# AssemblyAI-Community/MinImagen

Measured on NVIDIA H100. Metric: denoising steps/sec (SR256 U-Net, batch 32 per GPU per step), higher is better.
Workload: dtype f16 tensor-core operands, f32 accumulate / residual stream

## Files before the change

### minimagen_b200/csrc/conv_tc.cu

```cuda
#include "conv_tc.cuh"

#include <cuda_runtime.h>
#include <mutex>
#include <stdio.h>

#include "kernels.cuh"
#include "launch.cuh"
#include "ptx.cuh"
#include "sat_half.cuh"
#include "wgmma.cuh"

namespace mi {

namespace {

constexpr int kNumThreads = 384;
constexpr uint32_t kABytes = kConvBlockM * kConvBlockK * 2;
constexpr uint32_t kRingBudget = 192 * 1024;
constexpr uint32_t kAuxBytes = 512;
constexpr uint32_t kSmemMax = 227 * 1024;
constexpr int kProducerRegs = 40;
constexpr int kConsumerRegs = 232;
static_assert(128 * kProducerRegs + 256 * kConsumerRegs <= 65536, "register file overcommitted");
constexpr int kTurnBar = 2;
constexpr int kStatBar = 4;
constexpr uint32_t stat_scratch_bytes(int block_n) { return 2 * 4 * (block_n / 16 > 0 ? block_n / 16 : 1) * 2 * 8; }

template <int BLOCK_N>
struct Cfg {
    static constexpr uint32_t kBBytes = BLOCK_N * kConvBlockK * 2;
    static constexpr uint32_t kStageBytes = kABytes + kBBytes;
    static constexpr int kStages = (kRingBudget / kStageBytes) > 8 ? 8 : (kRingBudget / kStageBytes);
    static constexpr uint32_t kSmemBytes = kStages * kStageBytes + 1024  + kAuxBytes;
};

__device__ __forceinline__ float silu(float v) { return __fdividef(v, 1.0f + __expf(-v)); }

template <int BLOCK_N, bool GN>
__global__ void __launch_bounds__(kNumThreads, 1)
conv_wg_kernel(const __grid_constant__ CUtensorMap tmA, const __grid_constant__ CUtensorMap tmA2,
               const __grid_constant__ CUtensorMap tmB, const __grid_constant__ CUtensorMap tmX,
               const __grid_constant__ CUtensorMap tmX2, const __grid_constant__ ConvTcArgs args,
               const __grid_constant__ GnPrologueArgs gn) {
    using C = Cfg<BLOCK_N>;
    constexpr int STAGES = C::kStages;
    static_assert(2 * STAGES * 8 <= 256, "barrier block overlaps the GroupNorm scratch");
    constexpr bool PP = !GN && BLOCK_N <= 128;
    constexpr int HALVES = PP ? 2 : 1;

    extern __shared__ uint8_t smem_raw[];
    uint8_t* smem = reinterpret_cast<uint8_t*>((reinterpret_cast<uintptr_t>(smem_raw) + 1023) & ~uintptr_t(1023));
    uint64_t* bars = reinterpret_cast<uint64_t*>(smem + STAGES * C::kStageBytes);
    uint64_t* full_bar = bars;
    uint64_t* empty_bar = bars + STAGES;

    const int warp = threadIdx.x >> 5;
    const int lane = threadIdx.x & 31;
    const int wg = threadIdx.x >> 7;
    int* err = args.err_flag;

    if (threadIdx.x == 0) {
        ptx::prefetch_tensormap(&tmB);
        if (!GN) {
            ptx::prefetch_tensormap(&tmA);
            ptx::prefetch_tensormap(&tmA2);
        }
        for (int i = 0; i < STAGES; ++i) {
            ptx::mbar_init(&full_bar[i], GN ? 5 : 1);
            ptx::mbar_init(&empty_bar[i], PP ? 1 : 2);
        }
        ptx::fence_barrier_init();
    }
    __syncthreads();
    pdl_wait();

    const int num_tap_kb = args.num_taps * args.chunks_per_tap;
    const int num_kb = num_tap_kb + args.x_chunks;
    const int tiles_m = args.tiles_w * args.tiles_h * args.tiles_b;
    const int total_tiles = tiles_m * args.tiles_n;
    const int BW = 1 << args.bw_log2, BH = 1 << args.bh_log2;
    const int BB = kConvBlockM >> (args.bw_log2 + args.bh_log2);

    if (wg == 0) {
        if constexpr (!GN) {
            ptx::setmaxnreg_dec<kProducerRegs>();
            if (warp == 0) {
                int stage = 0;
                uint32_t phase = 0;
                for (int tile = blockIdx.x; tile < total_tiles; tile += gridDim.x) {
                    const int nt = tile % args.tiles_n;
                    const int mt = tile / args.tiles_n;
                    const int w0 = (mt % args.tiles_w) * BW;
                    const int h0 = ((mt / args.tiles_w) % args.tiles_h) * BH;
                    const int b0 = (mt / (args.tiles_w * args.tiles_h)) * BB;
                    const int n0 = nt * BLOCK_N;
                    for (int kb = 0; kb < num_kb; ++kb) {
                        ptx::mbar_wait(&empty_bar[stage], phase ^ 1, err, 100 + stage);
                        if (ptx::elect_one()) {
                            uint8_t* sa = smem + stage * C::kStageBytes;
                            uint8_t* sb = sa + kABytes;
                            ptx::mbar_arrive_expect_tx(&full_bar[stage], C::kStageBytes);
                            if (kb < num_tap_kb) {
                                const int t = kb / args.chunks_per_tap, j = kb - t * args.chunks_per_tap;
                                const int cw = w0 * args.in_stride + args.dw[t], ch = h0 * args.in_stride + args.dh[t];
                                if (j < args.a_split)
                                    ptx::tma_load_5d(&tmA, &full_bar[stage], sa, args.a_chan_off + j * kConvBlockK, cw, ch,
                                                     args.ph[t], b0);
                                else
                                    ptx::tma_load_5d(&tmA2, &full_bar[stage], sa,
                                                     args.a_chan_off2 + (j - args.a_split) * kConvBlockK, cw, ch, args.ph[t], b0);
                            } else {
                                const int jx = kb - num_tap_kb;
                                if (jx < args.x_split)
                                    ptx::tma_load_5d(&tmX, &full_bar[stage], sa, args.x_chan_off + jx * kConvBlockK, w0, h0, 0, b0);
                                else
                                    ptx::tma_load_5d(&tmX2, &full_bar[stage], sa,
                                                     args.x_chan_off2 + (jx - args.x_split) * kConvBlockK, w0, h0, 0, b0);
                            }
                            ptx::tma_load_2d(&tmB, &full_bar[stage], sb, kb * kConvBlockK, n0);
                        }
                        if (++stage == STAGES) { stage = 0; phase ^= 1; }
                    }
                }
                pdl_trigger();
            }
        } else {
            float* s_mean = reinterpret_cast<float*>(reinterpret_cast<uint8_t*>(bars) + 256);
            float* s_rstd = s_mean + 32;
            float* sA = reinterpret_cast<float*>(reinterpret_cast<uint8_t*>(bars) + kAuxBytes);
            const int tt = threadIdx.x;
            const int lq = tt & 7;
            const int prow = tt >> 3;
            const int C0 = gn.C0, C1 = gn.C1, Ctot = C0 + C1, Cg = Ctot / gn.groups;
            const int H = args.H, W = args.W;
            float* sB = sA + Ctot;
            int stage = 0;
            uint32_t phase = 0;
            int cur_b = -1;
            for (int tile = blockIdx.x; tile < total_tiles; tile += gridDim.x) {
                const int nt = tile % args.tiles_n;
                const int mt = tile / args.tiles_n;
                const int w0 = (mt % args.tiles_w) * BW;
                const int h0 = ((mt / args.tiles_w) % args.tiles_h) * BH;
                const int b = mt / (args.tiles_w * args.tiles_h);
                const int n0 = nt * BLOCK_N;
                if (b != cur_b) {
                    ptx::bar_sync(1, 128);
                    if (tt < gn.groups) {
                        const int g = tt;
                        double su = 0.0, sq = 0.0;
                        const int lo = g * Cg, hi = lo + Cg;
                        const int lo0 = min(lo, C0), hi0 = min(hi, C0);
                        for (int e = lo0 / 16; e < hi0 / 16; ++e) {
                            su += gn.stats0[((long long)b * (C0 / 16) + e) * 2];
                            sq += gn.stats0[((long long)b * (C0 / 16) + e) * 2 + 1];
                        }
                        const int lo1 = max(lo, C0) - C0, hi1 = max(hi, C0) - C0;
                        for (int e = lo1 / 16; e < hi1 / 16; ++e) {
                            su += (double)gn.scale1 * gn.stats1[((long long)b * (C1 / 16) + e) * 2];
                            sq += (double)gn.scale1 * (double)gn.scale1 * gn.stats1[((long long)b * (C1 / 16) + e) * 2 + 1];
                        }
                        const double n = (double)Cg * H * W;
                        const double mean = su / n;
                        double var = sq / n - mean * mean;
                        if (var < 0) var = 0;
                        s_mean[g] = (float)mean;
                        s_rstd[g] = (float)(1.0 / sqrt(var + (double)gn.eps));
                    }
                    ptx::bar_sync(1, 128);
                    for (int cc = tt; cc < Ctot; cc += 128) {
                        const int g = cc / Cg;
                        float a = s_rstd[g] * gn.gamma[cc];
                        float bb = gn.beta[cc] - s_mean[g] * a;
                        if (gn.scale_shift) {
                            const float sc = gn.scale_shift[(long long)b * gn.ss_ld + cc] + 1.0f;
                            const float shv = gn.scale_shift[(long long)b * gn.ss_ld + Ctot + cc];
                            a *= sc;
                            bb = bb * sc + shv;
                        }
                        if (cc >= C0) a *= gn.scale1;
                        sA[cc] = a;
                        sB[cc] = bb;
                    }
                    cur_b = b;
                    ptx::bar_sync(1, 128);
                }
                const long long img = (long long)b * H * W;
                for (int kb = 0; kb < num_kb; ++kb) {
                    const int t = kb / args.chunks_per_tap, j = kb - t * args.chunks_per_tap;
                    const int dh = args.dh[t], dw = args.dw[t];
                    const float* cA = sA + j * kConvBlockK + lq * 8;
                    const float* cB = sB + j * kConvBlockK + lq * 8;
                    const float4 a0 = *reinterpret_cast<const float4*>(cA), a1 = *reinterpret_cast<const float4*>(cA + 4);
                    const float4 b0 = *reinterpret_cast<const float4*>(cB), b1 = *reinterpret_cast<const float4*>(cB + 4);
                    const bool first = j < args.a_split;
                    const int Cs = first ? C0 : C1;
                    const float* src = (first ? gn.src0 + (long long)j * kConvBlockK
                                              : gn.src1 + (long long)(j - args.a_split) * kConvBlockK) + img * Cs + lq * 8;

                    ptx::mbar_wait(&empty_bar[stage], phase ^ 1, err, 600 + stage);
                    uint8_t* sa = smem + stage * C::kStageBytes;
                    if (warp == 0 && ptx::elect_one()) {
                        ptx::mbar_arrive_expect_tx(&full_bar[stage], C::kBBytes);
                        ptx::tma_load_2d(&tmB, &full_bar[stage], sa + kABytes, kb * kConvBlockK, n0);
                    }
                    float4 x0[8], x1[8];
                    bool ok[8];
#pragma unroll
                    for (int i = 0; i < 8; ++i) {
                        const int m = i * 16 + prow;
                        const int gw = w0 + (m & (BW - 1)) + dw;
                        const int gh = h0 + ((m >> args.bw_log2) & (BH - 1)) + dh;
                        ok[i] = gh >= 0 && gh < H && gw >= 0 && gw < W;
                        if (ok[i]) {
                            const float4* s4 = reinterpret_cast<const float4*>(src + ((long long)gh * W + gw) * Cs);
                            x0[i] = __ldg(s4);
                            x1[i] = __ldg(s4 + 1);
                        }
                    }
#pragma unroll
                    for (int i = 0; i < 8; ++i) {
                        const int m = i * 16 + prow;
                        uint4 o = make_uint4(0u, 0u, 0u, 0u);
                        if (ok[i]) {
                            const __half2 h0_ = sat_half2(silu(fmaf(x0[i].x, a0.x, b0.x)), silu(fmaf(x0[i].y, a0.y, b0.y)));
                            const __half2 h1_ = sat_half2(silu(fmaf(x0[i].z, a0.z, b0.z)), silu(fmaf(x0[i].w, a0.w, b0.w)));
                            const __half2 h2_ = sat_half2(silu(fmaf(x1[i].x, a1.x, b1.x)), silu(fmaf(x1[i].y, a1.y, b1.y)));
                            const __half2 h3_ = sat_half2(silu(fmaf(x1[i].z, a1.z, b1.z)), silu(fmaf(x1[i].w, a1.w, b1.w)));
                            o.x = *reinterpret_cast<const uint32_t*>(&h0_); o.y = *reinterpret_cast<const uint32_t*>(&h1_);
                            o.z = *reinterpret_cast<const uint32_t*>(&h2_); o.w = *reinterpret_cast<const uint32_t*>(&h3_);
                        }
                        *reinterpret_cast<uint4*>(sa + m * 128 + ((lq ^ (m & 7)) << 4)) = o;
                    }
                    ptx::fence_proxy_async_smem();
                    __syncwarp();
                    if (lane == 0) ptx::mbar_arrive(&full_bar[stage]);
                    if (++stage == STAGES) { stage = 0; phase ^= 1; }
                }
            }
            pdl_trigger();
        }
    } else {
        if constexpr (!GN) ptx::setmaxnreg_inc<kConsumerRegs>();
        const int cw = wg - 1;
        const int wq = warp & 3;
        const int cq = 2 * (lane & 3);
        float acc[HALVES][BLOCK_N / 2];
        int stage = 0;
        uint32_t phase = 0;
        auto skip = [&](int n) {
            stage += n % STAGES;
            phase ^= (uint32_t)(n / STAGES) & 1u;
            if (stage >= STAGES) { stage -= STAGES; phase ^= 1; }
        };
        if (PP) skip(cw * num_kb);
        int bw_r[2 * HALVES], bh_r[2 * HALVES], bb_r[2 * HALVES], bb_warp[HALVES];
#pragma unroll
        for (int h = 0; h < HALVES; ++h) {
            const int m_warp = (PP ? h : cw) * 64 + wq * 16;
            bb_warp[h] = m_warp >> (args.bw_log2 + args.bh_log2);
#pragma unroll
            for (int r = 0; r < 2; ++r) {
                const int m = m_warp + (lane >> 2) + 8 * r;
                bw_r[2 * h + r] = m & (BW - 1);
                bh_r[2 * h + r] = (m >> args.bw_log2) & (BH - 1);
                bb_r[2 * h + r] = m >> (args.bw_log2 + args.bh_log2);
            }
        }
        constexpr int NQ = BLOCK_N / 16 > 0 ? BLOCK_N / 16 : 1;
        const bool tile_stats = PP && args.stats != nullptr && BB == 1;
        double* st_red = reinterpret_cast<double*>(reinterpret_cast<uint8_t*>(bars) + kAuxBytes);
        const bool vec = args.out_sc == 1 && ((reinterpret_cast<uintptr_t>(args.out_f32) & 7) == 0) &&
                         ((reinterpret_cast<uintptr_t>(args.residual) & 7) == 0) &&
                         ((reinterpret_cast<uintptr_t>(args.out_f16) & 3) == 0);

        for (int tile = blockIdx.x + (PP ? cw : 0) * gridDim.x; tile < total_tiles; tile += (PP ? 2 : 1) * gridDim.x) {
            const int nt = tile % args.tiles_n;
            const int mt = tile / args.tiles_n;
            const int n0 = nt * BLOCK_N;
            if (PP && tile != (int)blockIdx.x) ptx::bar_sync(kTurnBar + cw, 256);
            int prev = -1;
            for (int kb = 0; kb < num_kb; ++kb) {
                ptx::mbar_wait(&full_bar[stage], phase, err, 300 + stage);
                const uint32_t sa = ptx::smem_u32(smem + stage * C::kStageBytes);
                const uint64_t db = ptx::make_sw128_desc(sa + kABytes);
                ptx::wg_fence();
#pragma unroll
                for (int k = 0; k < kConvBlockK / 16; ++k)
#pragma unroll
                    for (int h = 0; h < HALVES; ++h) {
                        const uint64_t da = ptx::make_sw128_desc(sa + (PP ? h : cw) * (64 * 128));
                        ptx::Wgmma<BLOCK_N, 0>::run(acc[h], da + 2 * k, db + 2 * k, (kb | k) != 0);
                    }
                ptx::wg_commit();
                ptx::wg_wait<1>();
                if (prev >= 0 && (threadIdx.x & 127) == 0) ptx::mbar_arrive(&empty_bar[prev]);
                prev = stage;
                if (++stage == STAGES) { stage = 0; phase ^= 1; }
            }
            if (PP && tile + (int)gridDim.x < total_tiles) ptx::bar_arrive(kTurnBar + (cw ^ 1), 256);
            if (PP) skip(num_kb);
            ptx::wg_wait<0>();
#pragma unroll
            for (int h = 0; h < HALVES; ++h) ptx::wg_fence_regs(acc[h]);
            if (prev >= 0 && (threadIdx.x & 127) == 0) ptx::mbar_arrive(&empty_bar[prev]);

            const int tw0 = (mt % args.tiles_w) * BW;
            const int th0 = ((mt / args.tiles_w) % args.tiles_h) * BH;
            const int tb0 = (mt / (args.tiles_w * args.tiles_h)) * BB;
            const bool fast = vec && n0 + BLOCK_N <= args.n_valid;
#pragma unroll
            for (int hf = 0; hf < HALVES; ++hf) {
                bool valid[2];
                long long pix[2];
#pragma unroll
                for (int r = 0; r < 2; ++r) {
                    const int w = tw0 + bw_r[2 * hf + r], h = th0 + bh_r[2 * hf + r], b = tb0 + bb_r[2 * hf + r];
                    valid[r] = (b < args.B) && (h < args.H) && (w < args.W);
                    pix[r] = (long long)b * args.out_sb + (long long)h * args.out_sh + (long long)w * args.out_sw;
                }
                const float* a = acc[hf];
                float st_s[BLOCK_N / 16 > 0 ? BLOCK_N / 16 : 1], st_q[BLOCK_N / 16 > 0 ? BLOCK_N / 16 : 1];
#pragma unroll
                for (int q = 0; q < BLOCK_N / 16; ++q) { st_s[q] = 0.f; st_q[q] = 0.f; }
#pragma unroll
                for (int j = 0; j < BLOCK_N / 8; ++j) {
                    const int n = n0 + 8 * j + cq;
                    if (fast) {
                        float2 bv = make_float2(0.f, 0.f);
                        if (args.bias) bv = __ldg(reinterpret_cast<const float2*>(args.bias + n));
#pragma unroll
                        for (int r = 0; r < 2; ++r) {
                            if (!valid[r]) continue;
                            const long long o = pix[r] + n;
                            float2 f = make_float2(a[4 * j + 2 * r] + bv.x, a[4 * j + 2 * r + 1] + bv.y);
                            if (args.residual) {
                                const float2 rv = *reinterpret_cast<const float2*>(args.residual + o);
                                f.x += rv.x; f.y += rv.y;
                            }
                            st_s[j >> 1] += f.x + f.y;
                            st_q[j >> 1] += f.x * f.x + f.y * f.y;
                            if (args.out_f32) *reinterpret_cast<float2*>(args.out_f32 + o) = f;
                            if (args.out_f16) *reinterpret_cast<__half2*>(args.out_f16 + o) = sat_half2(f.x, f.y);
                        }
                    } else {
#pragma unroll
                        for (int r = 0; r < 2; ++r) {
#pragma unroll
                            for (int e = 0; e < 2; ++e) {
                                if (!valid[r] || n + e >= args.n_valid) continue;
                                float f = a[4 * j + 2 * r + e] + (args.bias ? __ldg(args.bias + n + e) : 0.f);
                                const long long o = pix[r] + (long long)(n + e) * args.out_sc;
                                if (args.residual && args.out_sc == 1) f += args.residual[o];
                                st_s[j >> 1] += f;
                                st_q[j >> 1] += f * f;
                                if (args.out_f32) args.out_f32[o] = f;
                                if (args.out_f16) args.out_f16[o] = sat_half(f);
                            }
                        }
                    }
                }
                if (args.stats) {
                    const int b_img = tb0 + bb_warp[hf];
                    const bool any = __any_sync(0xffffffffu, valid[0] || valid[1]);
#pragma unroll
                    for (int q = 0; q < BLOCK_N / 16; ++q) {
#pragma unroll
                        for (int o = 1; o <= 16; o <<= 1) {
                            st_s[q] += __shfl_xor_sync(0xffffffffu, st_s[q], o);
                            st_q[q] += __shfl_xor_sync(0xffffffffu, st_q[q], o);
                        }
                        if (lane == 0 && tile_stats) {
                            double* r = st_red + ((cw * 4 + wq) * NQ + q) * 2;
                            r[0] = (hf == 0 ? 0.0 : r[0]) + (double)st_s[q];
                            r[1] = (hf == 0 ? 0.0 : r[1]) + (double)st_q[q];
                        } else if (lane == 0 && any) {
                            double* dst = args.stats + ((long long)b_img * args.stats_blocks + (n0 >> 4) + q) * 2;
                            atomicAdd(dst, (double)st_s[q]);
                            atomicAdd(dst + 1, (double)st_q[q]);
                        }
                    }
                }
            }
            if (tile_stats) {
                ptx::bar_sync(kStatBar + cw, 128);
                if (wq == 0 && lane < NQ) {
                    const double* r = st_red + (cw * 4 * NQ + lane) * 2;
                    double s = r[0], sq = r[1];
#pragma unroll
                    for (int w = 1; w < 4; ++w) { s += r[w * NQ * 2]; sq += r[w * NQ * 2 + 1]; }
                    double* dst = args.stats + ((long long)tb0 * args.stats_blocks + (n0 >> 4) + lane) * 2;
                    atomicAdd(dst, s);
                    atomicAdd(dst + 1, sq);
                }
                ptx::bar_sync(kStatBar + cw, 128);
            }
        }
    }
}


typedef CUresult (*PFN_encodeTiled)(CUtensorMap*, CUtensorMapDataType, cuuint32_t, void*, const cuuint64_t*,
                                    const cuuint64_t*, const cuuint32_t*, const cuuint32_t*, CUtensorMapInterleave,
                                    CUtensorMapSwizzle, CUtensorMapL2promotion, CUtensorMapFloatOOBfill);

PFN_encodeTiled get_encode() {
    static PFN_encodeTiled fn = nullptr;
    static std::once_flag once;
    std::call_once(once, [] {
        void* p = nullptr;
        cudaDriverEntryPointQueryResult q;
        if (cudaGetDriverEntryPoint("cuTensorMapEncodeTiled", &p, cudaEnableDefault, &q) == cudaSuccess &&
            q == cudaDriverEntryPointSuccess)
            fn = reinterpret_cast<PFN_encodeTiled>(p);
    });
    return fn;
}

int ilog2_exact(int v) {
    int l = 0;
    while ((1 << l) < v) ++l;
    return ((1 << l) == v) ? l : -1;
}

int num_sms_of_current_device() {
    int dev = 0;
    cudaGetDevice(&dev);
    static int cache[64] = {0};
    if (dev < 64 && cache[dev] != 0) return cache[dev];
    int n = 0;
    cudaDeviceGetAttribute(&n, cudaDevAttrMultiProcessorCount, dev);
    if (dev < 64) cache[dev] = n;
    return n;
}

void tile_geometry(int H, int W, int B, ConvTcArgs& a) {
    int BW = W >= 128 ? 128 : W;
    int BH = 128 / BW;
    if (BH > H) BH = H;
    const int BB = 128 / (BW * BH);
    a.bw_log2 = ilog2_exact(BW);
    a.bh_log2 = ilog2_exact(BH);
    a.tiles_w = (W + BW - 1) / BW;
    a.tiles_h = H / BH;
    a.tiles_b = (B + BB - 1) / BB;
    a.B = B; a.H = H; a.W = W;
}

int pick_block_n(int Cout, int tiles_m, int hint, int num_sms) {
    const int cands[5] = {256, 128, 64, 32, 16};
    if (hint < 0) hint = -hint;
    if (hint > 0 && Cout % hint == 0)
        for (int i = 0; i < 5; ++i)
            if (cands[i] == hint) return hint;
    int block_n = 16;
    for (int i = 0; i < 5; ++i) {
        if (Cout % cands[i] != 0) continue;
        block_n = cands[i];
        if (tiles_m * (Cout / cands[i]) >= num_sms || cands[i] <= 64) break;
    }
    return block_n;
}

CUresult encode_act(PFN_encodeTiled enc, CUtensorMap* m, const void* ptr, cuuint64_t channels, cuuint64_t ld, int W, int H,
                    int phases, int B, int in_stride, const ConvTcArgs& a) {
    const cuuint64_t IS = in_stride;
    const int BW = 1 << a.bw_log2, BH = 1 << a.bh_log2, BB = kConvBlockM >> (a.bw_log2 + a.bh_log2);
    cuuint64_t gdim[5] = {channels, (cuuint64_t)W * IS, (cuuint64_t)H * IS, (cuuint64_t)phases, (cuuint64_t)B};
    cuuint64_t gstr[4] = {ld * 2, (cuuint64_t)W * IS * ld * 2, (cuuint64_t)H * IS * W * IS * ld * 2,
                          (cuuint64_t)phases * H * IS * W * IS * ld * 2};
    cuuint32_t box[5] = {kConvBlockK, (cuuint32_t)(BW * IS), (cuuint32_t)(BH * IS), 1, (cuuint32_t)BB};
    cuuint32_t estr[5] = {1, (cuuint32_t)IS, (cuuint32_t)IS, 1, 1};
    return enc(m, CU_TENSOR_MAP_DATA_TYPE_FLOAT16, 5, const_cast<void*>(ptr), gdim, gstr, box, estr,
               CU_TENSOR_MAP_INTERLEAVE_NONE, CU_TENSOR_MAP_SWIZZLE_128B, CU_TENSOR_MAP_L2_PROMOTION_L2_256B,
               CU_TENSOR_MAP_FLOAT_OOB_FILL_NONE);
}

CUresult encode_weights(PFN_encodeTiled enc, CUtensorMap* m, const void* ptr, cuuint64_t K, int Cout, int block_n) {
    cuuint64_t gdim[2] = {K, (cuuint64_t)Cout};
    cuuint64_t gstr[1] = {K * 2};
    cuuint32_t box[2] = {kConvBlockK, (cuuint32_t)block_n};
    cuuint32_t estr[2] = {1, 1};
    return enc(m, CU_TENSOR_MAP_DATA_TYPE_FLOAT16, 2, const_cast<void*>(ptr), gdim, gstr, box, estr,
               CU_TENSOR_MAP_INTERLEAVE_NONE, CU_TENSOR_MAP_SWIZZLE_128B, CU_TENSOR_MAP_L2_PROMOTION_L2_256B,
               CU_TENSOR_MAP_FLOAT_OOB_FILL_NONE);
}

template <int BLOCK_N, bool GN>
int launch(const CUtensorMap& tmA, const CUtensorMap& tmA2, const CUtensorMap& tmB, const CUtensorMap& tmX,
           const CUtensorMap& tmX2, const ConvTcArgs& args, const GnPrologueArgs& gn, uint32_t extra_smem,
           cudaStream_t stream) {
    using C = Cfg<BLOCK_N>;
    static bool attr_set = false;
    if (!attr_set) {
        if (cudaFuncSetAttribute(conv_wg_kernel<BLOCK_N, GN>, cudaFuncAttributeMaxDynamicSharedMemorySize, kSmemMax) !=
            cudaSuccess)
            return -10;
        attr_set = true;
    }
    const int total_tiles = args.tiles_w * args.tiles_h * args.tiles_b * args.tiles_n;
    const int num_sms = num_sms_of_current_device();
    const int grid = total_tiles < num_sms ? total_tiles : num_sms;
    const uint32_t smem = C::kSmemBytes + (!GN && BLOCK_N <= 128 ? stat_scratch_bytes(BLOCK_N) : 0u) + extra_smem;
    launch_k(conv_wg_kernel<BLOCK_N, GN>, grid, kNumThreads, smem, stream, tmA, tmA2, tmB, tmX, tmX2, args, gn);
    return cudaGetLastError() == cudaSuccess ? 0 : -11;
}

}

PFN_tmaEncodeTiled get_tma_encode() { return get_encode(); }

const char* conv_tc_strerror(int code) {
    switch (code) {
        case 0: return "ok";
        case -1: return "conv_tc: C_in (per tap) must be a positive multiple of 64";
        case -2: return "conv_tc: C_out must be a multiple of 16";
        case -3: return "conv_tc: W must be a power of two >= 8 or a multiple of 128; H*W tiling unsupported";
        case -4: return "conv_tc: too many taps (max 16)";
        case -5: return "conv_tc: cuTensorMapEncodeTiled unavailable";
        case -6: return "conv_tc: tensor map encode failed (activations)";
        case -7: return "conv_tc: tensor map encode failed (weights)";
        case -8: return "conv_tc: pointer/stride alignment (16 B) violated";
        case -9: return "conv_tc: the folded 1x1 operand needs a stride-1 conv over one phase";
        case -10: return "conv_tc: cudaFuncSetAttribute(max dynamic smem) failed";
        case -11: return "conv_tc: kernel launch failed";
        default: return "conv_tc: unknown error";
    }
}

bool conv_tc_supported(int H, int W, int Cin, int Cout) {
    if (Cin <= 0 || Cin % kConvBlockK != 0 || Cout <= 0 || Cout % 16 != 0) return false;
    if (W >= 128) return true;
    if (ilog2_exact(W) < 3) return false;
    const int bh = 128 / W;
    if (H >= bh) return H % bh == 0;
    return ilog2_exact(H) >= 0;
}

int conv_tc_launch(const ConvTcProblem& p, cudaStream_t stream) {
    if (p.Cin <= 0 || p.Cin % kConvBlockK != 0) return -1;
    if (p.Cout % 16 != 0) return -2;
    if (p.num_taps < 1 || p.num_taps > kConvMaxTaps) return -4;
    if (!conv_tc_supported(p.H, p.W, p.Cin, p.Cout)) return -3;
    if ((reinterpret_cast<uintptr_t>(p.act) & 15) || (reinterpret_cast<uintptr_t>(p.wpacked) & 15) ||
        (p.lda % 8) != 0)
        return -8;
    PFN_encodeTiled enc = get_encode();
    if (!enc) return -5;

    ConvTcArgs a{};
    a.num_taps = p.num_taps;
    a.chunks_per_tap = p.Cin / kConvBlockK;
    tile_geometry(p.H, p.W, p.B, a);
    a.a_chan_off = p.a_chan_off;
    a.in_stride = p.in_stride == 2 ? 2 : 1;
    a.out_sb = p.out_sb; a.out_sh = p.out_sh; a.out_sw = p.out_sw;
    a.out_sc = p.out_sc > 0 ? p.out_sc : 1;
    a.n_valid = p.n_valid > 0 ? p.n_valid : p.Cout;
    a.out_f32 = p.out_f32; a.out_f16 = p.out_f16; a.bias = p.bias; a.residual = p.residual;
    a.err_flag = p.err_flag;
    a.stats = p.stats; a.stats_blocks = p.Cout / 16;
    for (int t = 0; t < p.num_taps; ++t) { a.dh[t] = p.dh[t]; a.dw[t] = p.dw[t]; a.ph[t] = p.ph[t]; }

    const int tiles_m = a.tiles_w * a.tiles_h * a.tiles_b;
    const int block_n = pick_block_n(p.Cout, tiles_m, p.block_n_hint, num_sms_of_current_device());
    a.tiles_n = p.Cout / block_n;

    CUtensorMap tmA, tmA2, tmB, tmX, tmX2;
    a.a_split = (p.act2 ? p.Cin1 : p.Cin) / kConvBlockK;
    a.a_chan_off2 = p.a_chan_off2;
    if (encode_act(enc, &tmA, p.act, p.a_channels, p.lda, p.W, p.H, p.phases, p.B, a.in_stride, a) != CUDA_SUCCESS) return -6;
    tmA2 = tmA;
    if (p.act2) {
        if (p.Cin1 <= 0 || p.Cin1 % kConvBlockK || p.Cin1 >= p.Cin || (p.lda2 % 8) || (reinterpret_cast<uintptr_t>(p.act2) & 15) ||
            a.in_stride != 1)
            return -8;
        if (encode_act(enc, &tmA2, p.act2, p.lda2, p.lda2, p.W, p.H, p.phases, p.B, 1, a) != CUDA_SUCCESS) return -6;
    }
    tmX = tmA; tmX2 = tmA;
    if (p.x_act) {
        if (p.phases != 1 || a.in_stride != 1) return -9;
        if (p.Cx <= 0 || p.Cx % kConvBlockK || (p.x_lda % 8) || (reinterpret_cast<uintptr_t>(p.x_act) & 15)) return -8;
        if (p.x_act2 && (p.Cx1 <= 0 || p.Cx1 % kConvBlockK || p.Cx1 >= p.Cx || (p.x_lda2 % 8) ||
                         (reinterpret_cast<uintptr_t>(p.x_act2) & 15)))
            return -8;
        a.x_chunks = p.Cx / kConvBlockK;
        a.x_split = (p.x_act2 ? p.Cx1 : p.Cx) / kConvBlockK;
        a.x_chan_off = p.x_chan_off; a.x_chan_off2 = p.x_chan_off2;
        if (encode_act(enc, &tmX, p.x_act, p.x_lda, p.x_lda, p.W, p.H, 1, p.B, 1, a) != CUDA_SUCCESS) return -6;
        tmX2 = tmX;
        if (p.x_act2 && encode_act(enc, &tmX2, p.x_act2, p.x_lda2, p.x_lda2, p.W, p.H, 1, p.B, 1, a) != CUDA_SUCCESS) return -6;
    }
    const cuuint64_t K = (cuuint64_t)p.num_taps * p.Cin + (p.x_act ? (cuuint64_t)p.Cx : 0);
    if (encode_weights(enc, &tmB, p.wpacked, K, p.Cout, block_n) != CUDA_SUCCESS) return -7;

    const GnPrologueArgs gn{};
    switch (block_n) {
        case 256: return launch<256, false>(tmA, tmA2, tmB, tmX, tmX2, a, gn, 0, stream);
        case 128: return launch<128, false>(tmA, tmA2, tmB, tmX, tmX2, a, gn, 0, stream);
        case 64: return launch<64, false>(tmA, tmA2, tmB, tmX, tmX2, a, gn, 0, stream);
        case 32: return launch<32, false>(tmA, tmA2, tmB, tmX, tmX2, a, gn, 0, stream);
        default: return launch<16, false>(tmA, tmA2, tmB, tmX, tmX2, a, gn, 0, stream);
    }
}


bool conv_gn_supported(int H, int W, int C0, int C1, int Cout, int groups) {
    const int C = C0 + C1;
    if (H <= 0 || W <= 0 || H % 32 || W % 8 || C0 <= 0 || C0 % 64 || C1 < 0 || C1 % 64 || Cout <= 0 || Cout % 128) return false;
    if (!conv_tc_supported(H, W, C, Cout) || H * W < kConvBlockM) return false;
    if (groups < 1 || groups > 32 || C % groups) return false;
    if (Cfg<128>::kSmemBytes + 8u * (uint32_t)C > kSmemMax) return false;
    return (C / groups) % 16 == 0;
}

int conv_gn_launch(const ConvGnProblem& p, cudaStream_t stream) {
    if (!conv_gn_supported(p.H, p.W, p.C0, p.C1, p.Cout, p.groups)) return -3;
    if (p.C1 && (!p.src1 || !p.stats1)) return -8;
    if (!p.src0 || !p.stats0 || !p.gamma || !p.beta) return -8;
    if ((reinterpret_cast<uintptr_t>(p.src0) & 15) || (reinterpret_cast<uintptr_t>(p.src1) & 15) ||
        (reinterpret_cast<uintptr_t>(p.wpacked) & 15))
        return -8;
    PFN_encodeTiled enc = get_encode();
    if (!enc) return -5;
    const int C = p.C0 + p.C1;

    ConvTcArgs a{};
    a.num_taps = 9;
    for (int t = 0; t < 9; ++t) { a.dh[t] = (int8_t)(t / 3 - 1); a.dw[t] = (int8_t)(t % 3 - 1); a.ph[t] = 0; }
    a.chunks_per_tap = C / kConvBlockK;
    a.a_split = p.C0 / kConvBlockK;
    a.in_stride = 1;
    tile_geometry(p.H, p.W, p.B, a);
    a.out_sb = (long long)p.H * p.W * p.Cout; a.out_sh = (long long)p.W * p.Cout; a.out_sw = p.Cout; a.out_sc = 1;
    a.n_valid = p.Cout;
    a.out_f32 = p.out_f32; a.out_f16 = p.out_f16; a.bias = p.bias; a.residual = p.residual; a.err_flag = p.err_flag;
    a.stats = p.out_stats; a.stats_blocks = p.Cout / 16;
    a.tiles_n = p.Cout / 128;

    GnPrologueArgs g{};
    g.src0 = p.src0; g.src1 = p.src1;
    g.C0 = p.C0; g.C1 = p.C1; g.groups = p.groups; g.scale1 = p.scale1; g.eps = p.eps;
    g.stats0 = p.stats0; g.stats1 = p.stats1; g.gamma = p.gamma; g.beta = p.beta;
    g.scale_shift = p.scale_shift; g.ss_ld = p.ss_ld;

    CUtensorMap tmB;
    if (encode_weights(enc, &tmB, p.wpacked, (cuuint64_t)9 * C, p.Cout, 128) != CUDA_SUCCESS) return -7;
    return launch<128, true>(tmB, tmB, tmB, tmB, tmB, a, g, 8u * (uint32_t)C, stream);
}

}
```

Measured before the change: 15.75.

## Add transposed 256-pixel conv tile for 128-channel outputs

```diff
diff --git a/minimagen_b200/csrc/conv_tc.cu b/minimagen_b200/csrc/conv_tc.cu
--- a/minimagen_b200/csrc/conv_tc.cu
+++ b/minimagen_b200/csrc/conv_tc.cu
@@ -36,7 +36,7 @@
 
 __device__ __forceinline__ float silu(float v) { return __fdividef(v, 1.0f + __expf(-v)); }
 
-template <int BLOCK_N, bool GN>
+template <int BLOCK_N, bool GN, bool TR = false>
 __global__ void __launch_bounds__(kNumThreads, 1)
 conv_wg_kernel(const __grid_constant__ CUtensorMap tmA, const __grid_constant__ CUtensorMap tmA2,
                const __grid_constant__ CUtensorMap tmB, const __grid_constant__ CUtensorMap tmX,
@@ -45,8 +45,10 @@
     using C = Cfg<BLOCK_N>;
     constexpr int STAGES = C::kStages;
     static_assert(2 * STAGES * 8 <= 256, "barrier block overlaps the GroupNorm scratch");
-    constexpr bool PP = !GN && BLOCK_N <= 128;
+    static_assert(!TR || (BLOCK_N == 256 && !GN), "the transposed tile is the cooperative 256-wide one");
+    constexpr bool PP = !GN && !TR && BLOCK_N <= 128;
     constexpr int HALVES = PP ? 2 : 1;
+    constexpr int TILE_PIX = TR ? BLOCK_N : kConvBlockM;
 
     extern __shared__ uint8_t smem_raw[];
     uint8_t* smem = reinterpret_cast<uint8_t*>((reinterpret_cast<uintptr_t>(smem_raw) + 1023) & ~uintptr_t(1023));
@@ -79,7 +81,7 @@
     const int tiles_m = args.tiles_w * args.tiles_h * args.tiles_b;
     const int total_tiles = tiles_m * args.tiles_n;
     const int BW = 1 << args.bw_log2, BH = 1 << args.bh_log2;
-    const int BB = kConvBlockM >> (args.bw_log2 + args.bh_log2);
+    const int BB = TILE_PIX >> (args.bw_log2 + args.bh_log2);
 
     if (wg == 0) {
         if constexpr (!GN) {
@@ -97,8 +99,8 @@
                     for (int kb = 0; kb < num_kb; ++kb) {
                         ptx::mbar_wait(&empty_bar[stage], phase ^ 1, err, 100 + stage);
                         if (ptx::elect_one()) {
-                            uint8_t* sa = smem + stage * C::kStageBytes;
-                            uint8_t* sb = sa + kABytes;
+                            uint8_t* sa = smem + stage * C::kStageBytes + (TR ? kABytes : 0);
+                            uint8_t* sb = smem + stage * C::kStageBytes + (TR ? 0 : kABytes);
                             ptx::mbar_arrive_expect_tx(&full_bar[stage], C::kStageBytes);
                             if (kb < num_tap_kb) {
                                 const int t = kb / args.chunks_per_tap, j = kb - t * args.chunks_per_tap;
@@ -308,6 +310,72 @@
             const int tw0 = (mt % args.tiles_w) * BW;
             const int th0 = ((mt / args.tiles_w) % args.tiles_h) * BH;
             const int tb0 = (mt / (args.tiles_w * args.tiles_h)) * BB;
+            if constexpr (TR) {
+                const int c0 = 64 * cw + 16 * wq + (lane >> 2);
+                const float bv[2] = {args.bias ? __ldg(args.bias + c0) : 0.f, args.bias ? __ldg(args.bias + c0 + 8) : 0.f};
+                const long long base = (long long)tb0 * args.out_sb + (long long)th0 * args.out_sh +
+                                       (long long)(tw0 + cq) * args.out_sw + c0;
+                float* const o32 = args.out_f32 ? args.out_f32 + base : nullptr;
+                __half* const o16 = args.out_f16 ? args.out_f16 + base : nullptr;
+                const float* const res = args.residual ? args.residual + base : nullptr;
+                const int sw = (int)args.out_sw, step = 8 * sw, wrap = (int)args.out_sh - (BW - 8) * sw;
+                float* a = acc[0];
+                int oj = 0;
+#pragma unroll
+                for (int j = 0; j < BLOCK_N / 8; ++j) {
+                    if (j > 0) oj += ((8 * j) & (BW - 1)) ? step : wrap;
+#pragma unroll
+                    for (int r = 0; r < 2; ++r)
+#pragma unroll
+                        for (int e = 0; e < 2; ++e) {
+                            float& f = a[4 * j + 2 * r + e];
+                            f += bv[r];
+                            if (res) f += res[oj + e * sw + 8 * r];
+                        }
+                }
+                const bool stats = args.stats != nullptr;
+                double su = 0.0, sq = 0.0;
+                oj = 0;
+#pragma unroll
+                for (int jj = 0; jj < BLOCK_N / 16; ++jj) {
+                    float s8 = 0.f, q8 = 0.f;
+#pragma unroll
+                    for (int j = 2 * jj; j < 2 * jj + 2; ++j) {
+                        if (j > 0) oj += ((8 * j) & (BW - 1)) ? step : wrap;
+#pragma unroll
+                        for (int r = 0; r < 2; ++r) {
+                            const float* f = a + 4 * j + 2 * r;
+#pragma unroll
+                            for (int e = 0; e < 2; ++e) {
+                                const int o = oj + e * sw + 8 * r;
+                                if (o32) o32[o] = f[e];
+                                if (o16) o16[o] = sat_half(f[e]);
+                            }
+                            if (stats) {
+                                s8 += f[0] + f[1];
+                                q8 += f[0] * f[0] + f[1] * f[1];
+                            }
+                        }
+                    }
+                    if (stats) {
+                        su += (double)s8;
+                        sq += (double)q8;
+                    }
+                }
+                if (stats) {
+#pragma unroll
+                    for (int o = 1; o <= 16; o <<= 1) {
+                        su += __shfl_xor_sync(0xffffffffu, su, o);
+                        sq += __shfl_xor_sync(0xffffffffu, sq, o);
+                    }
+                    if (lane == 0) {
+                        double* dst = args.stats + ((long long)tb0 * args.stats_blocks + (c0 >> 4)) * 2;
+                        atomicAdd(dst, su);
+                        atomicAdd(dst + 1, sq);
+                    }
+                }
+                continue;
+            }
             const bool fast = vec && n0 + BLOCK_N <= args.n_valid;
 #pragma unroll
             for (int hf = 0; hf < HALVES; ++hf) {
@@ -434,11 +502,11 @@
     return n;
 }
 
-void tile_geometry(int H, int W, int B, ConvTcArgs& a) {
-    int BW = W >= 128 ? 128 : W;
-    int BH = 128 / BW;
+void tile_geometry(int H, int W, int B, int tile_pix, ConvTcArgs& a) {
+    int BW = W >= tile_pix ? tile_pix : W;
+    int BH = tile_pix / BW;
     if (BH > H) BH = H;
-    const int BB = 128 / (BW * BH);
+    const int BB = tile_pix / (BW * BH);
     a.bw_log2 = ilog2_exact(BW);
     a.bh_log2 = ilog2_exact(BH);
     a.tiles_w = (W + BW - 1) / BW;
@@ -463,9 +531,9 @@
 }
 
 CUresult encode_act(PFN_encodeTiled enc, CUtensorMap* m, const void* ptr, cuuint64_t channels, cuuint64_t ld, int W, int H,
-                    int phases, int B, int in_stride, const ConvTcArgs& a) {
+                    int phases, int B, int in_stride, int tile_pix, const ConvTcArgs& a) {
     const cuuint64_t IS = in_stride;
-    const int BW = 1 << a.bw_log2, BH = 1 << a.bh_log2, BB = kConvBlockM >> (a.bw_log2 + a.bh_log2);
+    const int BW = 1 << a.bw_log2, BH = 1 << a.bh_log2, BB = tile_pix >> (a.bw_log2 + a.bh_log2);
     cuuint64_t gdim[5] = {channels, (cuuint64_t)W * IS, (cuuint64_t)H * IS, (cuuint64_t)phases, (cuuint64_t)B};
     cuuint64_t gstr[4] = {ld * 2, (cuuint64_t)W * IS * ld * 2, (cuuint64_t)H * IS * W * IS * ld * 2,
                           (cuuint64_t)phases * H * IS * W * IS * ld * 2};
@@ -486,14 +554,23 @@
                CU_TENSOR_MAP_FLOAT_OOB_FILL_NONE);
 }
 
-template <int BLOCK_N, bool GN>
+bool transposed_ok(const ConvTcProblem& p, const ConvTcArgs& a) {
+    if (p.Cout != 128 || a.n_valid != p.Cout || a.out_sc != 1) return false;
+    const int BW = p.W >= 256 ? 256 : p.W;
+    if (p.W % BW || ilog2_exact(BW) < 3 || BW * a.in_stride > 256) return false;
+    const int BH = 256 / BW;
+    if (BH * a.out_sh + BW * a.out_sw + p.Cout > INT32_MAX) return false;
+    return p.H % BH == 0 && BH * a.in_stride <= 256;
+}
+
+template <int BLOCK_N, bool GN, bool TR = false>
 int launch(const CUtensorMap& tmA, const CUtensorMap& tmA2, const CUtensorMap& tmB, const CUtensorMap& tmX,
            const CUtensorMap& tmX2, const ConvTcArgs& args, const GnPrologueArgs& gn, uint32_t extra_smem,
            cudaStream_t stream) {
     using C = Cfg<BLOCK_N>;
     static bool attr_set = false;
     if (!attr_set) {
-        if (cudaFuncSetAttribute(conv_wg_kernel<BLOCK_N, GN>, cudaFuncAttributeMaxDynamicSharedMemorySize, kSmemMax) !=
+        if (cudaFuncSetAttribute(conv_wg_kernel<BLOCK_N, GN, TR>, cudaFuncAttributeMaxDynamicSharedMemorySize, kSmemMax) !=
             cudaSuccess)
             return -10;
         attr_set = true;
@@ -501,8 +578,8 @@
     const int total_tiles = args.tiles_w * args.tiles_h * args.tiles_b * args.tiles_n;
     const int num_sms = num_sms_of_current_device();
     const int grid = total_tiles < num_sms ? total_tiles : num_sms;
-    const uint32_t smem = C::kSmemBytes + (!GN && BLOCK_N <= 128 ? stat_scratch_bytes(BLOCK_N) : 0u) + extra_smem;
-    launch_k(conv_wg_kernel<BLOCK_N, GN>, grid, kNumThreads, smem, stream, tmA, tmA2, tmB, tmX, tmX2, args, gn);
+    const uint32_t smem = C::kSmemBytes + (!GN && !TR && BLOCK_N <= 128 ? stat_scratch_bytes(BLOCK_N) : 0u) + extra_smem;
+    launch_k(conv_wg_kernel<BLOCK_N, GN, TR>, grid, kNumThreads, smem, stream, tmA, tmA2, tmB, tmX, tmX2, args, gn);
     return cudaGetLastError() == cudaSuccess ? 0 : -11;
 }
 
@@ -551,7 +628,6 @@
     ConvTcArgs a{};
     a.num_taps = p.num_taps;
     a.chunks_per_tap = p.Cin / kConvBlockK;
-    tile_geometry(p.H, p.W, p.B, a);
     a.a_chan_off = p.a_chan_off;
     a.in_stride = p.in_stride == 2 ? 2 : 1;
     a.out_sb = p.out_sb; a.out_sh = p.out_sh; a.out_sw = p.out_sw;
@@ -562,20 +638,28 @@
     a.stats = p.stats; a.stats_blocks = p.Cout / 16;
     for (int t = 0; t < p.num_taps; ++t) { a.dh[t] = p.dh[t]; a.dw[t] = p.dw[t]; a.ph[t] = p.ph[t]; }
 
+    const int num_sms = num_sms_of_current_device();
+    const int hint = p.block_n_hint < 0 ? -p.block_n_hint : p.block_n_hint;
+    const bool tr_ok = transposed_ok(p, a);
+    const bool tr = hint == 256 ? tr_ok
+                                : (hint == 0 || p.Cout % hint != 0) && tr_ok && (long long)p.B * p.H * p.W / 256 >= num_sms;
+    const int tile_pix = tr ? 256 : kConvBlockM;
+    tile_geometry(p.H, p.W, p.B, tile_pix, a);
     const int tiles_m = a.tiles_w * a.tiles_h * a.tiles_b;
-    const int block_n = pick_block_n(p.Cout, tiles_m, p.block_n_hint, num_sms_of_current_device());
+    const int block_n = tr ? 128 : pick_block_n(p.Cout, tiles_m, p.block_n_hint, num_sms);
     a.tiles_n = p.Cout / block_n;
 
     CUtensorMap tmA, tmA2, tmB, tmX, tmX2;
     a.a_split = (p.act2 ? p.Cin1 : p.Cin) / kConvBlockK;
     a.a_chan_off2 = p.a_chan_off2;
-    if (encode_act(enc, &tmA, p.act, p.a_channels, p.lda, p.W, p.H, p.phases, p.B, a.in_stride, a) != CUDA_SUCCESS) return -6;
+    if (encode_act(enc, &tmA, p.act, p.a_channels, p.lda, p.W, p.H, p.phases, p.B, a.in_stride, tile_pix, a) != CUDA_SUCCESS)
+        return -6;
     tmA2 = tmA;
     if (p.act2) {
         if (p.Cin1 <= 0 || p.Cin1 % kConvBlockK || p.Cin1 >= p.Cin || (p.lda2 % 8) || (reinterpret_cast<uintptr_t>(p.act2) & 15) ||
             a.in_stride != 1)
             return -8;
-        if (encode_act(enc, &tmA2, p.act2, p.lda2, p.lda2, p.W, p.H, p.phases, p.B, 1, a) != CUDA_SUCCESS) return -6;
+        if (encode_act(enc, &tmA2, p.act2, p.lda2, p.lda2, p.W, p.H, p.phases, p.B, 1, tile_pix, a) != CUDA_SUCCESS) return -6;
     }
     tmX = tmA; tmX2 = tmA;
     if (p.x_act) {
@@ -587,14 +671,17 @@
         a.x_chunks = p.Cx / kConvBlockK;
         a.x_split = (p.x_act2 ? p.Cx1 : p.Cx) / kConvBlockK;
         a.x_chan_off = p.x_chan_off; a.x_chan_off2 = p.x_chan_off2;
-        if (encode_act(enc, &tmX, p.x_act, p.x_lda, p.x_lda, p.W, p.H, 1, p.B, 1, a) != CUDA_SUCCESS) return -6;
+        if (encode_act(enc, &tmX, p.x_act, p.x_lda, p.x_lda, p.W, p.H, 1, p.B, 1, tile_pix, a) != CUDA_SUCCESS) return -6;
         tmX2 = tmX;
-        if (p.x_act2 && encode_act(enc, &tmX2, p.x_act2, p.x_lda2, p.x_lda2, p.W, p.H, 1, p.B, 1, a) != CUDA_SUCCESS) return -6;
+        if (p.x_act2 &&
+            encode_act(enc, &tmX2, p.x_act2, p.x_lda2, p.x_lda2, p.W, p.H, 1, p.B, 1, tile_pix, a) != CUDA_SUCCESS)
+            return -6;
     }
     const cuuint64_t K = (cuuint64_t)p.num_taps * p.Cin + (p.x_act ? (cuuint64_t)p.Cx : 0);
     if (encode_weights(enc, &tmB, p.wpacked, K, p.Cout, block_n) != CUDA_SUCCESS) return -7;
 
     const GnPrologueArgs gn{};
+    if (tr) return launch<256, false, true>(tmA, tmA2, tmB, tmX, tmX2, a, gn, 0, stream);
     switch (block_n) {
         case 256: return launch<256, false>(tmA, tmA2, tmB, tmX, tmX2, a, gn, 0, stream);
         case 128: return launch<128, false>(tmA, tmA2, tmB, tmX, tmX2, a, gn, 0, stream);
@@ -631,7 +718,7 @@
     a.chunks_per_tap = C / kConvBlockK;
     a.a_split = p.C0 / kConvBlockK;
     a.in_stride = 1;
-    tile_geometry(p.H, p.W, p.B, a);
+    tile_geometry(p.H, p.W, p.B, kConvBlockM, a);
     a.out_sb = (long long)p.H * p.W * p.Cout; a.out_sh = (long long)p.W * p.Cout; a.out_sw = p.Cout; a.out_sc = 1;
     a.n_valid = p.Cout;
     a.out_f32 = p.out_f32; a.out_f16 = p.out_f16; a.bias = p.bias; a.residual = p.residual; a.err_flag = p.err_flag;
```

New measurement: 16.59 (median of 6 runs). +5.3%, better.
